# mcarrickscott/modarith

Measured on AMD Instinct MI355X. Metric: 256-bit modmul/s (2^255-19), higher is better.
Workload: dtype u64; 1 GPU; batched modmul 2^255-19, 5x51-bit limbs, 2^24 elements per GPU, limb-interleaved SoA, tiles of 4096 elements [n/4096][5][4096]; elements_per_gpu=16777216, placement_policy=single placement, no probe

## Files before the change

### include/modarith_amd.h

```cpp
#ifndef MODARITH_AMD_H
#define MODARITH_AMD_H

#include <stddef.h>
#include <stdint.h>

#ifdef __cplusplus
extern "C" {
#endif

typedef uint64_t ma_spint;

int modarith_amd_abi_version(void);
const char *modarith_amd_last_error(void);
int modarith_amd_status(void);
void modarith_amd_clear_status(void);
int modarith_amd_thread_status(void);
void modarith_amd_clear_thread_status(void);
int modarith_amd_device_count(void);
int modarith_amd_set_device(int dev);
int modarith_amd_malloc(void **dptr, size_t bytes);
int modarith_amd_free(void *dptr);
int modarith_amd_memcpy_h2d(void *dst, const void *src, size_t bytes, void *stream);
int modarith_amd_memcpy_d2h(void *dst, const void *src, size_t bytes, void *stream);
int modarith_amd_sync(void *stream);
int modarith_amd_stream_create(void **stream);
int modarith_amd_stream_destroy(void *stream);
int modarith_amd_stream_wait(void *stream, void *other);
int modarith_amd_host_alloc(void **hptr, size_t bytes);
int modarith_amd_host_free(void *hptr);
int modarith_amd_aos_to_soa(const ma_spint *aos, ma_spint *soa, size_t n, int nlimbs, size_t ld, void *stream);
int modarith_amd_soa_to_aos(const ma_spint *soa, ma_spint *aos, size_t n, int nlimbs, size_t ld, void *stream);
size_t modarith_amd_recommended_ld(size_t n);
size_t modarith_amd_recommended_ld_for(size_t n, int nlimbs);
size_t modarith_amd_batch_words(size_t n, int nlimbs, size_t ld);
int modarith_amd_scratch_trim(size_t keep_bytes);
int modarith_amd_sclk_probe(uint64_t *out, unsigned delay_us, unsigned window_us, void *stream);
int modarith_amd_wall_clock_khz(void);
const char *modarith_amd_last_launch(void);
int modarith_amd_field_info(const char *prime, int *nlimbs, int *radix, int *nbits, int *nbytes, int *montgomery);

#define MODARITH_AMD_ABI 2

#define MODARITH_AMD_DECLARE(P)                                                                                         \
                                \
    ma_spint prop_##P##_ct(ma_spint *n);            \
    ma_spint flatten_##P##_ct(ma_spint *n);                                                                             \
    ma_spint modfsb_##P##_ct(ma_spint *n);                                                                              \
    void modadd_##P##_ct(const ma_spint *a, const ma_spint *b, ma_spint *n);                                            \
    void modsub_##P##_ct(const ma_spint *a, const ma_spint *b, ma_spint *n);                                            \
    void modneg_##P##_ct(const ma_spint *b, ma_spint *n);                                                               \
    void modmli_##P##_ct(const ma_spint *a, int b, ma_spint *c);                                                        \
    void modmul_##P##_ct(const ma_spint *a, const ma_spint *b, ma_spint *c);                                            \
    void modsqr_##P##_ct(const ma_spint *a, ma_spint *c);                                                               \
    void modcpy_##P##_ct(const ma_spint *a, ma_spint *c);                                                               \
    void modnsqr_##P##_ct(ma_spint *a, int n);                                                                          \
    void modpro_##P##_ct(const ma_spint *w, ma_spint *z);                                                               \
    void modinv_##P##_ct(const ma_spint *x, const ma_spint *h, ma_spint *z);                         \
    int modqr_##P##_ct(const ma_spint *h, const ma_spint *x);                                        \
// ... 230 lines not shown
```

### modarith_amd/_lib.py

```python
from __future__ import annotations

import ctypes
import os
from ctypes import c_char_p, c_int, c_size_t, c_uint, c_void_p

HERE = os.path.dirname(os.path.abspath(__file__))
LIB_PATH = os.environ.get("MA_LIB", os.path.join(HERE, "libmodarith_amd.so"))
PRIMES = ("X25519", "NIST256", "X448",
          "NIST521", "PM266", "PM383", "NUMS256W", "NIST384", "NIST224", "SECP256K1M", "NIST256Q", "ED25519Q", "ED448Q",
          "C2065", "PM336", "PM512", "GM270", "GM240", "GM360", "GM480", "GM384", "GM512", "TWEEDLE", "SIDH434", "SIDH503",
          "SECP256K1", "C41417", "ED248", "ED376", "ED500",
          "SIDH610", "SIDH751", "MFP4", "MFP7", "MFP1973", "CSIDH512", "GM378",
          "PM383M", "PM266M", "PM336M", "C41417M", "PM512M", "M607")
LADDERS = ("X25519", "X448")
CURVES = {"ed25519": (5, 32), "ed448": (8, 56), "nist256": (5, 32), "nist384": (7, 48), "nist521": (9, 66), "secp256k1": (5, 32), "nums256w": (5, 32), "nums256e": (5, 32), "ed248": (5, 32), "ed376": (7, 48), "ed500": (9, 64)}
ED_BATCH_FUNCS = ("mul", "mul2", "mul2_exact", "ran", "add", "sub", "cpy", "dbl", "neg", "inf", "gen", "cof", "affine", "cmp", "isinf", "set", "get")
FUSED_CURVES = ("ed25519", "ed448", "nist256", "secp256k1")
FUSED2_CURVES = ("ed25519", "ed448", "nist256", "secp256k1")
FUSEDG_CURVES = ("nist256", "secp256k1", "ed25519", "ed448")
FUSEDG2_CURVES = ("nist256", "secp256k1", "ed25519", "ed448")
FUSED_FUNCS = (("rfc7748_X25519_base_batch", "rfc7748_X448_base_batch") + tuple("ecn_%s_mulgen_get_batch" % c for c in FUSEDG_CURVES)
               + tuple("ecn_%s_mulgen2_get_%s" % (c, f) for c in FUSEDG2_CURVES for f in ("batch", "workspace_bytes")) + tuple("ecn_%s_mul_get_%s" % (c, f) for c in FUSED_CURVES for f in ("batch", "workspace_bytes"))
               + tuple("ecn_%s_mul2_get_%s" % (c, f) for c in FUSED2_CURVES for f in ("batch", "workspace_bytes")))
ED_SCALAR_FUNCS = ("mul2", "ran", "get", "set", "inf", "isinf", "neg", "add", "sub", "dbl", "gen", "mul", "cmp", "affine", "cpy", "cof",
# ... 32 lines not shown
    "modsign": [_P, _P, c_size_t, c_size_t, _P],
    "modlimbs": [_P, _P, c_size_t, c_size_t, _P],
    "modcmp": [_P, _P, _P, c_size_t, c_size_t, _P],
    "modzer": [_P, c_size_t, c_size_t, _P],
    "modone": [_P, c_size_t, c_size_t, _P],
    "modint": [c_int, _P, c_size_t, c_size_t, _P],
    "mod2r": [c_uint, _P, c_size_t, c_size_t, _P],
    "modcmv": [_P, _P, _P, c_size_t, c_size_t, _P],
    "modcsw": [_P, _P, _P, c_size_t, c_size_t, _P],
    "modimp": [_P, _P, _P, c_size_t, c_size_t, _P],
    "modexp": [_P, _P, c_size_t, c_size_t, _P],
    "time_protocol": [c_int, _P, _P, _P, ctypes.c_long, c_size_t, c_size_t, _P],
    "moduniform": [ctypes.c_ulonglong, ctypes.c_ulonglong, c_size_t, c_int, _P, c_size_t, c_size_t, _P],
}
BATCH_FUNCS = tuple(_SIG)
SCALAR_FUNCS = ("prop", "flatten", "modfsb", "modadd", "modsub", "modneg", "modmli", "modmul", "modsqr", "modcpy", "modnsqr",
                "modpro", "modinv", "modqr", "modsqrt", "nres", "redc", "modis1", "modis0", "modzer", "modone", "modint", "modcmv",
                "modcsw", "modshl", "modshr", "modhaf", "mod2r", "modexp", "modimp", "modsign", "modcmp")
UTIL_FUNCS = ("modarith_amd_abi_version", "modarith_amd_last_error", "modarith_amd_device_count",
              "modarith_amd_set_device", "modarith_amd_malloc", "modarith_amd_free", "modarith_amd_memcpy_h2d",
              "modarith_amd_memcpy_d2h", "modarith_amd_sync", "modarith_amd_aos_to_soa", "modarith_amd_soa_to_aos",
              "modarith_amd_stream_create", "modarith_amd_stream_destroy", "modarith_amd_stream_wait", "modarith_amd_host_alloc", "modarith_amd_host_free",
              "modarith_amd_field_info", "modarith_amd_recommended_ld", "modarith_amd_recommended_ld_for", "modarith_amd_batch_words", "modarith_amd_scratch_trim",
              "modarith_amd_last_launch", "modarith_amd_status", "modarith_amd_clear_status", "modarith_amd_thread_status", "modarith_amd_clear_thread_status", "modarith_amd_sclk_probe", "modarith_amd_wall_clock_khz")

W32_PRIMES = ("X25519", "NIST256", "X448")
W32_ABSENT = ("modmuls", "modadd_lazy", "modsub_lazy", "modneg_lazy", "time_protocol")
_SIG_W32 = {fn: args for fn, args in _SIG.items() if fn not in W32_ABSENT}
W32_BATCH_FUNCS = tuple(_SIG_W32)
W32_SCALAR_FUNCS = SCALAR_FUNCS
W32_UTIL_FUNCS = ("modarith_amd_w32_field_info", "modarith_amd_w32_aos_to_soa", "modarith_amd_w32_soa_to_aos", "modarith_amd_w32_batch_words")
W32_CURVES = {"ed25519": (9, 32), "nist256": (9, 32), "ed448": (16, 56)}
W32_ED_BATCH_FUNCS = tuple(f for f in ED_BATCH_FUNCS if f != "mul2_exact")
W32_ED_SCALAR_FUNCS = ED_SCALAR_FUNCS


def _declare_curve(lib, C: str, funcs=ED_BATCH_FUNCS) -> None:
    g = lambda f: getattr(lib, "ecn_%s_%s" % (C, f))
    g("mul_workspace_bytes").argtypes = [c_size_t]
    g("mul_workspace_bytes").restype = c_size_t
    g("mul_batch").argtypes = [_P, _P, c_size_t, c_size_t, _P, c_size_t, _P]
    g("mul2_batch").argtypes = [_P, _P, _P, _P, _P, c_size_t, c_size_t, _P, c_size_t, _P]
    if "mul2_exact" in funcs:
        g("mul2_exact_batch").argtypes = [_P, _P, _P, _P, _P, c_size_t, c_size_t, _P, c_size_t, _P]
    g("ran_batch").argtypes = [c_int, _P, c_size_t, c_size_t, _P]
    for f in ("add", "sub", "cpy"):
        g(f + "_batch").argtypes = [_P, _P, c_size_t, c_size_t, _P]
# ... 91 lines not shown
    lib.modarith_amd_free.argtypes = [_P]
    lib.modarith_amd_memcpy_h2d.argtypes = [_P, _P, c_size_t, _P]
    lib.modarith_amd_memcpy_d2h.argtypes = [_P, _P, c_size_t, _P]
    lib.modarith_amd_sync.argtypes = [_P]
    lib.modarith_amd_stream_create.argtypes = [ctypes.POINTER(c_void_p)]
    lib.modarith_amd_stream_destroy.argtypes = [_P]
    lib.modarith_amd_stream_wait.argtypes = [_P, _P]
    lib.modarith_amd_host_alloc.argtypes = [ctypes.POINTER(c_void_p), c_size_t]
    lib.modarith_amd_host_free.argtypes = [_P]
    lib.modarith_amd_recommended_ld.argtypes = [c_size_t]
    lib.modarith_amd_recommended_ld.restype = c_size_t
    lib.modarith_amd_recommended_ld_for.argtypes = [c_size_t, c_int]
    lib.modarith_amd_recommended_ld_for.restype = c_size_t
    lib.modarith_amd_batch_words.argtypes = [c_size_t, c_int, c_size_t]
    lib.modarith_amd_batch_words.restype = c_size_t
    lib.modarith_amd_scratch_trim.argtypes = [c_size_t]
    lib.modarith_amd_scratch_trim.restype = c_int
    lib.modarith_amd_last_launch.restype = c_char_p
    lib.modarith_amd_status.restype = c_int
    lib.modarith_amd_clear_status.restype = None
    lib.modarith_amd_sclk_probe.argtypes = [_P, ctypes.c_uint, ctypes.c_uint, _P]
    lib.modarith_amd_sclk_probe.restype = c_int
    lib.modarith_amd_wall_clock_khz.restype = c_int
    _lib = lib
    return lib


_plugins = {}


def load_plugin(tag: str, path: str = None, wl: int = 64) -> ctypes.CDLL:
    if (tag, wl) in _plugins:
        return _plugins[tag, wl]
    if wl not in (64, 32):
        raise ValueError("word length must be 64 or 32")
    load()
    if path is None:
        from .generate import plugin_path
        path = plugin_path(tag, wl=wl)
    if not os.path.exists(path):
        raise RuntimeError("modarith_amd: no plug-in for %r (%s) -- generate it with `python -m modarith_amd.generate %s <prime>`. "
                           "There is no CPU fallback." % (tag, path, "64" if wl == 64 else "w32"))
    lib = ctypes.CDLL(path)
    for fn, args in (_SIG if wl == 64 else _SIG_W32).items():
        f = getattr(lib, "%s_%s%s_batch" % (fn, tag, "" if wl == 64 else "_w32"))
        f.argtypes = args
# ... 46 lines not shown
```

### modarith_amd/csrc/capi_common.h

```cpp
#pragma once
#include <hip/hip_runtime.h>
#include <mutex>
#include <stddef.h>
#include <stdint.h>
#include <stdio.h>
#include <stdlib.h>
#include <string>

namespace ma {

void set_error(const std::string& msg);
int check_launch(const char* what);
int max_blocks();
int max_blocks_tiled();
int ladder_block();
bool force_fast();
bool force_exact();
bool inv_simul();
bool ladder_split();
int scratch_trim(size_t keep_bytes);
bool ladder_use_field();

inline unsigned grid_for(size_t nthreads, int block = 256, bool tiled = false) {
    size_t b = (nthreads + (size_t)block - 1) / (size_t)block;
    size_t cap = (size_t)(tiled ? max_blocks_tiled() : max_blocks());
    if (b > cap) b = cap;
    if (b < 1) b = 1;
    return (unsigned)b;
}

inline bool aligned16(const void* p) { return (reinterpret_cast<uintptr_t>(p) & 15u) == 0; }

void fail(const char* what, hipError_t e);
int sticky_status();
void clear_sticky_status();
int thread_status();
void clear_thread_status();

struct Staging {
    static constexpr int MAX_DEVICES = 64;
    std::mutex mu[MAX_DEVICES];
    unsigned char* dev[MAX_DEVICES] = {};
    static constexpr size_t BYTES = 512 * 1024;
    unsigned char* get(int d);
};
Staging& staging();
struct StageBase {
    std::unique_lock<std::mutex> lock;
    unsigned char* base = nullptr;
    size_t used = 0;
    bool bad = false;
    struct Src { const unsigned char* p; size_t b; } src[8];
// ... 30 lines not shown
```

### modarith_amd/csrc/capi_common.hip

```cpp
#include "../../include/modarith_amd.h"
#include "capi_common.h"
#include "kernels.h"
#include <atomic>
#include <string.h>

namespace ma {

static thread_local std::string g_err;
static thread_local const char* g_last_launch = "";

void set_error(const std::string& msg) { g_err = msg; }

int check_launch(const char* what) {
    g_last_launch = what;
    hipError_t e = hipGetLastError();
    if (e != hipSuccess) {
        set_error(std::string(what) + ": " + hipGetErrorString(e));
        return (int)e;
    }
    return 0;
}

static int env_int(const char* name, int dflt, int lo, int hi) {
    const char* s = getenv(name);
// ... 16 lines not shown
    static int v = env_int("MA_LADDER_BLOCK", 64, 64, 256) / 64 * 64;
    return v;
}

bool force_fast() {
    static bool v = [] { const char* s = getenv("MA_FORCE_FAST"); return s && *s == '1'; }();
    return v;
}
bool force_exact() {
    static bool v = [] { const char* s = getenv("MA_FORCE_EXACT"); return s && *s == '1'; }();
    return v;
}
bool inv_simul() {
    static bool v = [] { const char* s = getenv("MA_INV_SIMUL"); return !(s && *s == '0'); }();
    return v;
}
bool ladder_split() {
    static bool v = [] { const char* s = getenv("MA_LADDER_SPLIT"); return !(s && *s == '0'); }();
    return v;
}
bool ladder_use_field() {
    static bool v = [] { const char* s = getenv("MA_LADDER_IMPL"); return s && strcmp(s, "field") == 0; }();
    return v;
}

static std::atomic<int> g_sticky{0};
static thread_local int t_sticky = 0;
int thread_status() { return t_sticky; }
void clear_thread_status() { t_sticky = 0; }
void fail(const char* what, hipError_t e) {
    set_error(std::string(what) + " failed: " + hipGetErrorString(e));
    int zero = 0;
    const int code = e == hipSuccess ? (int)hipErrorUnknown : (int)e;
    g_sticky.compare_exchange_strong(zero, code);
    if (t_sticky == 0) t_sticky = code;
    (void)hipGetLastError();
}
int sticky_status() { return g_sticky.load(); }
void clear_sticky_status() { g_sticky.store(0); }

unsigned char* Staging::get(int d) {
    if (!dev[d]) {
        static const bool test_fail = [] { const char* s = getenv("MA_TEST_STAGING_FAIL"); return s && *s == '1'; }();
        hipError_t e = test_fail ? hipErrorOutOfMemory : hipMalloc((void**)&dev[d], BYTES);
        if (e != hipSuccess) {
            dev[d] = nullptr;
// ... 218 lines not shown
}

extern "C" {

int modarith_amd_abi_version(void) { return MODARITH_AMD_ABI; }
const char* modarith_amd_last_error(void) { return g_err.c_str(); }
const char* modarith_amd_last_launch(void) { return g_last_launch; }
int modarith_amd_status(void) { return sticky_status(); }
void modarith_amd_clear_status(void) { clear_sticky_status(); }
int modarith_amd_thread_status(void) { return thread_status(); }
void modarith_amd_clear_thread_status(void) { clear_thread_status(); }
int modarith_amd_wall_clock_khz(void) {
    int d = 0, khz = 0;
    if (hipGetDevice(&d) != hipSuccess || hipDeviceGetAttribute(&khz, hipDeviceAttributeWallClockRate, d) != hipSuccess) { (void)hipGetLastError(); return 0; }
    return khz;
}
int modarith_amd_sclk_probe(uint64_t* out, unsigned delay_us, unsigned window_us, void* st) {
    const int khz = modarith_amd_wall_clock_khz();
    if (khz <= 0) { set_error("sclk_probe: no wall-clock rate for this device"); return (int)hipErrorNotSupported; }
    k_sclk_probe<<<1, 64, 0, (hipStream_t)st>>>(out, (uint64_t)delay_us * (uint64_t)khz / 1000, (uint64_t)window_us * (uint64_t)khz / 1000);
    return check_launch("sclk_probe");
}
int modarith_amd_scratch_trim(size_t keep_bytes) { return scratch_trim(keep_bytes); }
size_t modarith_amd_recommended_ld(size_t n) { return n >= 2 * (size_t)4096 ? (size_t)4096 : n; }
size_t modarith_amd_recommended_ld_for(size_t n, int nlimbs) {
    const size_t t = nlimbs >= 8 ? (size_t)8192 : (size_t)4096;
    return n >= 2 * t ? t : modarith_amd_recommended_ld(n);
}
size_t modarith_amd_batch_words(size_t n, int nlimbs, size_t ld) {
    if (nlimbs < 1 || ld == 0) return 0;
    if (ld >= n) return (size_t)nlimbs * ld;
    return (n + ld - 1) / ld * ld * (size_t)nlimbs;
}
int modarith_amd_device_count(void) {
    int n = 0;
    if (hipGetDeviceCount(&n) != hipSuccess) return 0;
    return n;
}
int modarith_amd_set_device(int dev) { return wrap(hipSetDevice(dev), "hipSetDevice"); }
int modarith_amd_malloc(void** dptr, size_t bytes) { return wrap(hipMalloc(dptr, bytes), "hipMalloc"); }
int modarith_amd_free(void* dptr) { return wrap(hipFree(dptr), "hipFree"); }
int modarith_amd_memcpy_h2d(void* dst, const void* src, size_t bytes, void* stream) {
    return wrap(hipMemcpyAsync(dst, src, bytes, hipMemcpyHostToDevice, (hipStream_t)stream), "hipMemcpyAsync(h2d)");
}
int modarith_amd_memcpy_d2h(void* dst, const void* src, size_t bytes, void* stream) {
    return wrap(hipMemcpyAsync(dst, src, bytes, hipMemcpyDeviceToHost, (hipStream_t)stream), "hipMemcpyAsync(d2h)");
// ... 62 lines not shown
```

### modarith_amd/csrc/capi_field.inc

```

namespace {
bool make_ld(size_t n, size_t ld, Ld* L, const char* what) {
    if (ld >= n) { *L = Ld(ld); return true; }
    if (ld < 128 || (ld & (ld - 1)) != 0) {
        set_error(std::string(what) + ": a limb stride below n selects the tiled layout and must be a power of two >= 128");
        return false;
    }
    *L = Ld(ld, (unsigned)__builtin_ctzll((unsigned long long)ld));
    return true;
}
#define GRID(x) grid_for((x), BLOCK, L.s != 63)
#define MA_LD(what)                                                  \
    Ld L;                                                            \
    if (!make_ld(n, ld, &L, what)) return (int)hipErrorInvalidValue;

uintptr_t U(const void* p) { return reinterpret_cast<uintptr_t>(p); }
int pick_ept(size_t n, size_t ld, uintptr_t addr) {
    for (int e = ept_cap(); e > 1; e >>= 1)
        if (n >= (size_t)e && ld % e == 0 && (addr & (e * sizeof(spint) - 1)) == 0) return e;
    return 1;
}
template <int E> using Width = std::integral_constant<int, E>;
#ifdef MA_W32_EPT_MAX
constexpr int EPT_COMPILED = MA_W32_EPT_MAX;
#else
constexpr int EPT_COMPILED = 4;
#endif
template <class Go>
int launch_stream(size_t n, size_t ld, uintptr_t addr, const char* what, Go go) {
    if (n == 0) return 0;
    MA_LD(what)
    const int ept = pick_ept(n, ld, addr), sb = std::min(stream_block(), stream_block_max(ept));
    const size_t nt = n / ept, done = nt * ept;
    const unsigned grid = grid_for(nt, sb, L.s != 63);
    if (ept == 4) { if constexpr (MA_WL == 32 && EPT_COMPILED >= 4) go(Width<4>{}, grid, sb, 0, nt, L); }
    else if (ept == 2) { if constexpr (EPT_COMPILED >= 2) go(Width<2>{}, grid, sb, 0, nt, L); }
    else go(Width<1>{}, grid, sb, 0, nt, L);
    if (done < n) go(Width<1>{}, 1u, BLOCK, L.off<NL>(done), n - done, Ld(L.ld));
    return check_launch(what);
}
template <class Op, int E> using OpAt = typename std::conditional<E == 1, typename ScalarOp<Op>::type, Op>::type;
template <class Op>
int launch_binary(const spint* a, const spint* b, spint* c, size_t n, size_t ld, void* stream, const char* what) {
    return launch_stream(n, ld, U(a) | U(b) | U(c), what, [=](auto W, unsigned grid, int block, size_t o, size_t cnt, Ld l) {
        constexpr int E = decltype(W)::value;
        k_binary<P, OpAt<Op, E>, E><<<grid, block, 0, (hipStream_t)stream>>>(a + o, b + o, c + o, cnt, l, l, l);
    });
}
template <class Op>
int launch_unary(const spint* a, spint* c, size_t n, size_t ld, void* stream, const char* what) {
    return launch_stream(n, ld, U(a) | U(c), what, [=](auto W, unsigned grid, int block, size_t o, size_t cnt, Ld l) {
        constexpr int E = decltype(W)::value;
        k_unary<P, OpAt<Op, E>, E><<<grid, block, 0, (hipStream_t)stream>>>(a + o, c + o, cnt, l, l);
    });
}
template <class Op>
int launch_unary_heavy(const spint* a, spint* c, size_t n, size_t ld, void* stream, const char* what) {
    if (n == 0) return 0;
    MA_LD(what)
    k_unary_heavy<P, Op><<<GRID(n), BLOCK, 0, (hipStream_t)stream>>>(a, c, n, L, L);
    return check_launch(what);
}
int modinv_each(const spint* x, spint* z, size_t n, size_t ld, void* st);
bool inv_may_share();

struct Stage : StageBase {
    template <class T>
    T* put(const T* host, size_t count) {
        T* d = reinterpret_cast<T*>(take(count * sizeof(T)));
        if (host) h2d(d, host, count * sizeof(T));
        return d;
    }
    template <class T>
    void get(T* host, const T* dev, size_t count) { d2h(host, dev, count * sizeof(T)); }
};
}

extern "C" {

int BATCH(modadd)(const spint* a, const spint* b, spint* c, size_t n, size_t ld, void* st) { return launch_binary<OpAdd<P>>(a, b, c, n, ld, st, MA_WHAT("modadd")); }
int BATCH(modsub)(const spint* a, const spint* b, spint* c, size_t n, size_t ld, void* st) { return launch_binary<OpSub<P>>(a, b, c, n, ld, st, MA_WHAT("modsub")); }
int BATCH(modneg)(const spint* b, spint* c, size_t n, size_t ld, void* st) { return launch_unary<OpNeg<P>>(b, c, n, ld, st, MA_WHAT("modneg")); }
int BATCH(modcpy)(const spint* a, spint* c, size_t n, size_t ld, void* st) { return launch_unary<OpCpy<P>>(a, c, n, ld, st, MA_WHAT("modcpy")); }
int BATCH(modmli)(const spint* a, int b, spint* c, size_t n, size_t ld, void* st) {
    return launch_stream(n, ld, U(a) | U(c), MA_WHAT("modmli"), [=](auto W, unsigned grid, int block, size_t o, size_t cnt, Ld l) {
        k_mli<P, decltype(W)::value><<<grid, block, 0, (hipStream_t)st>>>(a + o, b, c + o, cnt, l, l);
    });
}

constexpr size_t INV_SIMUL_LANES = 16384;
constexpr size_t INV_SIMUL_MIN = 32768;
int BATCH(modinv)(const spint* x, const spint* h, spint* z, size_t n, size_t ld, void* st) {
    if (n == 0) return 0;
    MA_LD(MA_WHAT("modinv"))
    if constexpr (INV_SIMUL)
    if (h == nullptr && n >= INV_SIMUL_MIN && inv_simul() && inv_may_share()) {
        hipStream_t s = (hipStream_t)st;
        size_t rounds = (n + INV_SIMUL_LANES - 1) / INV_SIMUL_LANES;
        if (rounds > 64) rounds = 64;
        const size_t lanes = (n + rounds - 1) / rounds;
        const unsigned grid = (unsigned)((lanes + BLOCK - 1) / BLOCK);
        if (x != z) {
            k_inv_simul<P><<<grid, BLOCK, 0, s>>>(x, z, z, n, lanes, (int)rounds, L, L, L);
            return check_launch(MA_WHAT2("modinv", "simultaneous"));
        }
        hipStreamCaptureStatus cs = hipStreamCaptureStatusNone;
        if (s == nullptr || (hipStreamIsCapturing(s, &cs) == hipSuccess && cs == hipStreamCaptureStatusNone)) {
            if (spint* ws = static_cast<spint*>(scratch_alloc(n * NL * sizeof(spint), s))) {
                k_inv_simul<P><<<grid, BLOCK, 0, s>>>(x, z, ws, n, lanes, (int)rounds, L, L, Ld(n));
// ... 296 lines not shown
```

### modarith_amd/csrc/capi_prime.inc

```
#include "../../include/modarith_amd.h"
#include "capi_common.h"
#include "kernels.h"
#include "ladder.h"
#ifdef MA_LADDER_FE26
#include "fe26.h"
#endif
#ifdef MA_LADDER_FE28
#include "fe28.h"
#endif
#include <string.h>
#include <algorithm>

#define MA_CAT3_(a, b, c) a##_##b##_##c
#define MA_CAT3(a, b, c) MA_CAT3_(a, b, c)
#define BATCH(fn) MA_CAT3(fn, MA_NAME, batch)
#define SCALAR(fn) MA_CAT3(fn, MA_NAME, ct)

namespace {
using namespace ma;
using P = MA_P;
constexpr int NL = P::N;
constexpr int NB = P::NBYTES;
#define MA_WHAT(fn) fn
#define MA_WHAT2(fn, how) fn "(" how ")"
int ept_cap() { return 2; }
int stream_block() { return BLOCK; }
constexpr bool INV_SIMUL = NL <= 9 && P::RADIX <= 60;
}
#include "capi_field.inc"

namespace {
int modinv_each(const spint* x, spint* z, size_t n, size_t ld, void* st) {
    if (force_fast() && P::SPLIT > 0) return launch_unary_heavy<OpInv<P, true>>(x, z, n, ld, st, "modinv(fast)");
    if (force_exact() || P::SPLIT == 0) return launch_unary_heavy<OpInv<P>>(x, z, n, ld, st, "modinv(exact)");
    return launch_unary_heavy<OpAutoUnary<P, OpInv>>(x, z, n, ld, st, "modinv");
}
bool inv_may_share() { return !force_exact(); }
template <int EPT, bool AUTO>
void launch_shared(const spint* a, const Elem<P>& b0, spint* c, size_t nt, Ld L, unsigned grid, hipStream_t s) {
    k_mul_shared<P, EPT, AUTO><<<grid, BLOCK, 0, s>>>(a, b0, c, nt, L, L);
}
}

extern "C" {

int BATCH(modadd_lazy)(const ma_spint* a, const ma_spint* b, ma_spint* c, size_t n, size_t ld, void* st) { return launch_binary<OpAddLazy<P>>(a, b, c, n, ld, st, "modadd_lazy"); }
int BATCH(modsub_lazy)(const ma_spint* a, const ma_spint* b, ma_spint* c, size_t n, size_t ld, void* st) { return launch_binary<OpSubLazy<P>>(a, b, c, n, ld, st, "modsub_lazy"); }
int BATCH(modneg_lazy)(const ma_spint* b, ma_spint* c, size_t n, size_t ld, void* st) { return launch_unary<OpNegLazy<P>>(b, c, n, ld, st, "modneg_lazy"); }
int BATCH(modmul)(const ma_spint* a, const ma_spint* b, ma_spint* c, size_t n, size_t ld, void* st) {
    if (force_fast() && P::SPLIT > 0) return launch_binary<OpMul<P, true>>(a, b, c, n, ld, st, "modmul(fast)");
    if (force_exact() || P::SPLIT == 0) return launch_binary<OpMul<P>>(a, b, c, n, ld, st, "modmul(exact)");
    return launch_binary<OpMulAuto<P>>(a, b, c, n, ld, st, "modmul");
}
int BATCH(modsqr)(const ma_spint* a, ma_spint* c, size_t n, size_t ld, void* st) {
    if (force_fast() && P::SPLIT > 0) return launch_unary<OpSqr<P, true>>(a, c, n, ld, st, "modsqr(fast)");
    if (force_exact() || P::SPLIT == 0) return launch_unary<OpSqr<P>>(a, c, n, ld, st, "modsqr(exact)");
    return launch_unary<OpSqrAuto<P>>(a, c, n, ld, st, "modsqr");
}
int BATCH(nres)(const ma_spint* a, ma_spint* c, size_t n, size_t ld, void* st) {
    if (force_fast() && P::SPLIT > 0) return launch_unary<OpNres<P, true>>(a, c, n, ld, st, "nres(fast)");
    if (force_exact() || P::SPLIT == 0 || !P::MONTGOMERY) return launch_unary<OpNres<P>>(a, c, n, ld, st, "nres(exact)");
    return launch_unary<OpNresAuto<P>>(a, c, n, ld, st, "nres");
}
// ... 15 lines not shown
        return launch_unary_heavy<OpAutoUnary<P, OpSqrt>>(x, r, n, ld, st, "modsqrt");
    }
    k_sqrt_h<P, false><<<GRID(n), BLOCK, 0, (hipStream_t)st>>>(x, h, r, nullptr, n, L);
    return check_launch("modsqrt(h)");
}
int BATCH(modqr)(const ma_spint* h, const ma_spint* x, int* out, size_t n, size_t ld, void* st) {
    if (n == 0) return 0;
    MA_LD("modqr")
    if (h == nullptr) k_inplace<P, K_MODQR><<<GRID(n), BLOCK, 0, (hipStream_t)st>>>(const_cast<ma_spint*>(x), out, n, L);
    else k_sqrt_h<P, true><<<GRID(n), BLOCK, 0, (hipStream_t)st>>>(x, h, nullptr, out, n, L);
    return check_launch("modqr");
}

int BATCH(modmuls)(const ma_spint* a, const ma_spint* b0_host, ma_spint* c, size_t n, size_t ld, void* st) {
    if (n == 0) return 0;
    Elem<P> b0;
    bool b_ok = P::SPLIT > 0 && !force_exact();
    for (int i = 0; i < NL; i++) {
        b0.l[i] = b0_host[i];
        if (P::RADIX + 2 < 64 && (b0_host[i] >> ((P::RADIX + 2) & 63)) != 0) b_ok = false;
    }
    MA_LD("modmuls")
    hipStream_t s = (hipStream_t)st;
    if (n >= 2 && ld % 2 == 0 && aligned16(a) && aligned16(c)) {
        size_t nt = n / 2;
        if (b_ok) launch_shared<2, true>(a, b0, c, nt, L, GRID(nt), s);
        else launch_shared<2, false>(a, b0, c, nt, L, GRID(nt), s);
        const size_t o = L.off<NL>(n - 1);
        if (n & 1) launch_shared<1, false>(a + o, b0, c + o, 1, Ld(L.ld), 1, s);
    } else {
        launch_shared<1, false>(a, b0, c, n, L, GRID(n), s);
    }
    return check_launch("modmuls");
}

int BATCH(time_protocol)(int kind, const ma_spint* x, const ma_spint* y, ma_spint* z, long outer, size_t n, size_t ld, void* st) {
    if (n == 0) return 0;
    MA_LD("time_protocol")
    hipStream_t s = (hipStream_t)st;
    if (kind < 0 || kind > 2) { set_error("time_protocol: kind must be 0, 1 or 2"); return (int)hipErrorInvalidValue; }
    const int policy = (P::SPLIT == 0 || force_exact()) ? 0 : (force_fast() ? 1 : 2);
#define MA_TIME_LAUNCH(KIND, POL) k_time<P, KIND, POL><<<GRID(n), BLOCK, 0, s>>>(x, y, z, outer, n, L)
    if (policy == 0) { if (kind == 0) MA_TIME_LAUNCH(0, 0); else if (kind == 1) MA_TIME_LAUNCH(1, 0); else MA_TIME_LAUNCH(2, 0); }
    else if (policy == 1) { if (kind == 0) MA_TIME_LAUNCH(0, 1); else if (kind == 1) MA_TIME_LAUNCH(1, 1); else MA_TIME_LAUNCH(2, 1); }
    else { if (kind == 0) MA_TIME_LAUNCH(0, 2); else if (kind == 1) MA_TIME_LAUNCH(1, 2); else MA_TIME_LAUNCH(2, 2); }
#undef MA_TIME_LAUNCH
    return check_launch("time_protocol");
}

#ifdef MA_LADDER_A24
#define LADDER_BATCH_(name) rfc7748_##name##_batch
#define LADDER_BATCH(name) LADDER_BATCH_(name)
#define LADDER_SCALAR_(name) rfc7748_##name
#define LADDER_SCALAR(name) LADDER_SCALAR_(name)
// ... 93 lines not shown
```

### modarith_amd/csrc/kernels.h

```cpp
#pragma once
#include "field.h"

namespace MA_NS {

constexpr int BLOCK = 256;
constexpr int stream_block_max(int ept) { return MA_WL == 32 && ept == 1 ? 512 : BLOCK; }
__device__ __forceinline__ size_t stream_threads() { if constexpr (MA_WL == 32) return blockDim.x; else return BLOCK; }

template <int EPT> struct VecOf { typedef spint type __attribute__((ext_vector_type(EPT))); };
template <> struct VecOf<1> { typedef spint type; };
typedef VecOf<2>::type spint2;
#ifndef MA_NONTEMPORAL
#define MA_NONTEMPORAL 1
#endif
template <class T> __device__ __forceinline__ T ld_stream(const T* p) {
#if MA_NONTEMPORAL
    return __builtin_nontemporal_load(p);
#else
    return *p;
#endif
}
template <class T> __device__ __forceinline__ void st_stream(T* p, T v) {
#if MA_NONTEMPORAL
    __builtin_nontemporal_store(v, p);
#else
    *p = v;
#endif
}

struct Ld {
    size_t ld;
    unsigned s;
    __host__ __device__ Ld(size_t ld_ = 0) : ld(ld_), s(63) {}
    __host__ __device__ Ld(size_t ld_, unsigned s_) : ld(ld_), s(s_) {}
    template <int N>
    __host__ __device__ __forceinline__ size_t off(size_t j) const { return (((j >> s) * (size_t)N) << s) + (j & ((((size_t)1) << s) - 1)); }
};

template <class P, int EPT>
__device__ __forceinline__ void load_soa(const spint* base, Ld L, size_t t, spint (*x)[P::N]) {
    static_assert(EPT == 1 || EPT == 2 || (EPT == 4 && MA_WL == 32), "one or two elements per lane, four of 32-bit limbs");
    const spint* p = base + L.template off<P::N>((size_t)EPT * t);
    if constexpr (EPT == 1) {
        static_for<0, P::N>([&](auto I) { x[0][I] = ld_stream(p + (size_t)I * L.ld); });
    } else {
        using V = typename VecOf<EPT>::type;
        static_for<0, P::N>([&](auto I) {
            V v = ld_stream(reinterpret_cast<const V*>(p + (size_t)I * L.ld));
            static_for<0, EPT>([&](auto E) { constexpr int e = E; x[e][I] = v[e]; });
        });
    }
}
template <class P, int EPT>
__device__ __forceinline__ void store_soa(spint* base, Ld L, size_t t, spint (*x)[P::N]) {
    spint* p = base + L.template off<P::N>((size_t)EPT * t);
    if constexpr (EPT == 1) {
        static_for<0, P::N>([&](auto I) { st_stream(p + (size_t)I * L.ld, x[0][I]); });
    } else {
        using V = typename VecOf<EPT>::type;
        static_for<0, P::N>([&](auto I) {
            V v;
            static_for<0, EPT>([&](auto E) { constexpr int e = E; v[e] = x[e][I]; });
            st_stream(reinterpret_cast<V*>(p + (size_t)I * L.ld), v);
        });
    }
}

#if MA_WL == 64
#define MA_POLICY_OP template <class P, bool FAST = false>
#define MA_POLICY_FIELD Field<P, FAST>
#else
#define MA_POLICY_OP template <class P>
#define MA_POLICY_FIELD Field<P>
#endif
template <class P> using FieldVoted = Field<P, (P::SPLIT > 0)>;
MA_POLICY_OP struct OpMul { static MA_DEV void apply(const spint* a, const spint* b, spint* c) { MA_POLICY_FIELD::modmul(a, b, c); } };
template <class P> struct OpAdd { static MA_DEV void apply(const spint* a, const spint* b, spint* c) { Field<P>::modadd(a, b, c); } };
template <class P> struct OpSub { static MA_DEV void apply(const spint* a, const spint* b, spint* c) { Field<P>::modsub(a, b, c); } };
template <class P> struct OpAddLazy { static MA_DEV void apply(const spint* a, const spint* b, spint* c) { Field<P>::modadd_lazy(a, b, c); } };
template <class P> struct OpSubLazy { static MA_DEV void apply(const spint* a, const spint* b, spint* c) { Field<P>::modsub_lazy(a, b, c); } };
template <class P> MA_DEV bool in_split_contract(const spint* a) {
    if constexpr (P::RADIX + 2 >= 64) {
        return true;
    } else {
        spint m = 0;
        static_for<0, P::N>([&](auto I) { m |= a[I]; });
        return (m >> (P::RADIX + 2)) == 0;
    }
// ... 55 lines not shown
    spint t[F::N];
    F::redc(z, t);
    F::nres(t, z);
}
MA_POLICY_OP struct OpInv {
    static MA_DEV void apply(const spint* a, spint* c) {
        MA_POLICY_FIELD::modinv(a, nullptr, c);
        inv_normalise<MA_POLICY_FIELD>(c);
    }
};
MA_POLICY_OP struct OpSqrt { static MA_DEV void apply(const spint* a, spint* c) { MA_POLICY_FIELD::modsqrt(a, nullptr, c); } };
MA_POLICY_OP struct OpPro { static MA_DEV void apply(const spint* a, spint* c) { MA_POLICY_FIELD::modpro(a, c); } };
template <class P, template <class, bool> class Op> struct OpAutoUnary {
    static MA_DEV void apply(const spint* a, spint* c) {
        if constexpr (P::SPLIT > 0) {
            if (__all(in_split_contract<P>(a))) { Op<P, true>::apply(a, c); return; }
        }
        Op<P, false>::apply(a, c);
    }
};

template <class P, class Op, int EPT>
__global__ __launch_bounds__(stream_block_max(EPT)) void k_binary(const spint* a, const spint* b,
                                                                  spint* c, size_t nthreads, Ld lda, Ld ldb, Ld ldc) {
    for (size_t t = (size_t)blockIdx.x * stream_threads() + threadIdx.x; t < nthreads; t += (size_t)gridDim.x * stream_threads()) {
        spint x[EPT][P::N], y[EPT][P::N], z[EPT][P::N];
        load_soa<P, EPT>(a, lda, t, x);
        load_soa<P, EPT>(b, ldb, t, y);
        Op::apply(x[0], y[0], z[0]);
        if constexpr (EPT >= 2) Op::apply(x[1], y[1], z[1]);
        if constexpr (EPT == 4) { Op::apply(x[2], y[2], z[2]); Op::apply(x[3], y[3], z[3]); }
        store_soa<P, EPT>(c, ldc, t, z);
    }
}

template <class P> constexpr int heavy_waves() { return (MA_WL == 32 || P::N <= 5) ? 3 : 1; }
template <class P, class Op>
__global__ __launch_bounds__(BLOCK) __attribute__((amdgpu_waves_per_eu(heavy_waves<P>())))
void k_unary_heavy(const spint* a, spint* c, size_t nthreads, Ld lda, Ld ldc) {
    for (size_t t = (size_t)blockIdx.x * BLOCK + threadIdx.x; t < nthreads; t += (size_t)gridDim.x * BLOCK) {
        spint x[1][P::N], z[1][P::N];
        load_soa<P, 1>(a, lda, t, x);
        Op::apply(x[0], z[0]);
        store_soa<P, 1>(c, ldc, t, z);
    }
}

template <class P, class Op, int EPT>
__global__ __launch_bounds__(stream_block_max(EPT)) void k_unary(const spint* a, spint* c, size_t nthreads,
                                                                 Ld lda, Ld ldc) {
    for (size_t t = (size_t)blockIdx.x * stream_threads() + threadIdx.x; t < nthreads; t += (size_t)gridDim.x * stream_threads()) {
        spint x[EPT][P::N], z[EPT][P::N];
        load_soa<P, EPT>(a, lda, t, x);
        Op::apply(x[0], z[0]);
        if constexpr (EPT >= 2) Op::apply(x[1], z[1]);
        if constexpr (EPT == 4) { Op::apply(x[2], z[2]); Op::apply(x[3], z[3]); }
        store_soa<P, EPT>(c, ldc, t, z);
    }
}

template <class P> struct Elem { spint l[P::N]; };
template <class P, bool AUTO>
MA_DEV void mul_shared_one(const spint* x, const spint* b, spint* z) {
    if constexpr (AUTO && P::SPLIT > 0) {
        if (__all(in_split_contract<P>(x))) { Field<P, true>::modmul(x, b, z); return; }
    }
    Field<P, false>::modmul(x, b, z);
}
template <class P, int EPT, bool AUTO>
__global__ __launch_bounds__(BLOCK) void k_mul_shared(const spint* a, Elem<P> b0, spint* c,
                                                      size_t nthreads, Ld lda, Ld ldc) {
    for (size_t t = (size_t)blockIdx.x * BLOCK + threadIdx.x; t < nthreads; t += (size_t)gridDim.x * BLOCK) {
        spint x[EPT][P::N], z[EPT][P::N];
        load_soa<P, EPT>(a, lda, t, x);
        static_assert(EPT == 1 || EPT == 2, "one or two elements per lane");
        mul_shared_one<P, AUTO>(x[0], b0.l, z[0]);
        if constexpr (EPT == 2) mul_shared_one<P, AUTO>(x[1], b0.l, z[1]);
        store_soa<P, EPT>(c, ldc, t, z);
    }
}

template <class P, int EPT>
__global__ __launch_bounds__(stream_block_max(EPT)) void k_mli(const spint* a, int b, spint* c, size_t nthreads,
                                                               Ld lda, Ld ldc) {
    for (size_t t = (size_t)blockIdx.x * stream_threads() + threadIdx.x; t < nthreads; t += (size_t)gridDim.x * stream_threads()) {
        spint x[EPT][P::N], z[EPT][P::N];
        load_soa<P, EPT>(a, lda, t, x);
        Field<P>::modmli(x[0], b, z[0]);
        if constexpr (EPT >= 2) Field<P>::modmli(x[1], b, z[1]);
        if constexpr (EPT == 4) { Field<P>::modmli(x[2], b, z[2]); Field<P>::modmli(x[3], b, z[3]); }
        store_soa<P, EPT>(c, ldc, t, z);
    }
}

template <class P>
__global__ __launch_bounds__(BLOCK) void k_nsqr(spint* a, int k, size_t n, Ld ld) {
    for (size_t t = (size_t)blockIdx.x * BLOCK + threadIdx.x; t < n; t += (size_t)gridDim.x * BLOCK) {
        spint x[1][P::N];
        load_soa<P, 1>(a, ld, t, x);
        if constexpr (MA_WL == 32) {
            Field<P>::modnsqr(x[0], k);
        } else {
#pragma unroll 1
            for (int i = 0; i < k; i++) {
                bool fast = false;
                if constexpr (P::SPLIT > 0) fast = __all(in_split_contract<P>(x[0]));
                if (fast) Field<P, true>::modsqr(x[0], x[0]); else Field<P, false>::modsqr(x[0], x[0]);
            }
        }
        store_soa<P, 1>(a, ld, t, x);
    }
}

template <class P>
__global__ __launch_bounds__(BLOCK) void k_inv_h(const spint* xs, const spint* hs,
// ... 347 lines not shown
```

Baseline: 54.94 billion modmul/s.

## Alternate sweep direction per call and keep the tail chunks cache-resident

Streaming kernels (binary, unary, mli, shared-multiply) now walk block-sized chunks in a direction that flips on every call, per device. By default the last ~192 MiB of chunks use ordinary temporal loads and stores instead of nontemporal ones. The intent is that the data touched last stays in the last-level cache, so the next reversed call starts on cached data and cuts DRAM traffic for memory-bound batched modmul. The benefit depends on back-to-back calls over the same buffers. The default budget is tied to a guess about cache capacity. Per-thread control flow gets slightly more complex.

```diff
diff --git a/include/modarith_amd.h b/include/modarith_amd.h
--- a/include/modarith_amd.h
+++ b/include/modarith_amd.h
@@ -34,6 +34,12 @@
 size_t modarith_amd_recommended_ld_for(size_t n, int nlimbs);
 size_t modarith_amd_batch_words(size_t n, int nlimbs, size_t ld);
 int modarith_amd_scratch_trim(size_t keep_bytes);
+int modarith_amd_set_sweep(int mode);
+int modarith_amd_get_sweep(void);
+int modarith_amd_set_sweep_policy(int policy);
+int modarith_amd_get_sweep_policy(void);
+int modarith_amd_set_sweep_keep_mib(int mib);
+int modarith_amd_get_sweep_keep_mib(void);
 int modarith_amd_sclk_probe(uint64_t *out, unsigned delay_us, unsigned window_us, void *stream);
 int modarith_amd_wall_clock_khz(void);
 const char *modarith_amd_last_launch(void);
diff --git a/modarith_amd/_lib.py b/modarith_amd/_lib.py
--- a/modarith_amd/_lib.py
+++ b/modarith_amd/_lib.py
@@ -78,7 +78,9 @@
               "modarith_amd_memcpy_d2h", "modarith_amd_sync", "modarith_amd_aos_to_soa", "modarith_amd_soa_to_aos",
               "modarith_amd_stream_create", "modarith_amd_stream_destroy", "modarith_amd_stream_wait", "modarith_amd_host_alloc", "modarith_amd_host_free",
               "modarith_amd_field_info", "modarith_amd_recommended_ld", "modarith_amd_recommended_ld_for", "modarith_amd_batch_words", "modarith_amd_scratch_trim",
-              "modarith_amd_last_launch", "modarith_amd_status", "modarith_amd_clear_status", "modarith_amd_thread_status", "modarith_amd_clear_thread_status", "modarith_amd_sclk_probe", "modarith_amd_wall_clock_khz")
+              "modarith_amd_last_launch", "modarith_amd_status", "modarith_amd_clear_status", "modarith_amd_thread_status", "modarith_amd_clear_thread_status", "modarith_amd_sclk_probe", "modarith_amd_wall_clock_khz",
+              "modarith_amd_set_sweep", "modarith_amd_get_sweep", "modarith_amd_set_sweep_policy", "modarith_amd_get_sweep_policy",
+              "modarith_amd_set_sweep_keep_mib", "modarith_amd_get_sweep_keep_mib")
 
 W32_PRIMES = ("X25519", "NIST256", "X448")
 W32_ABSENT = ("modmuls", "modadd_lazy", "modsub_lazy", "modneg_lazy", "time_protocol")
@@ -216,6 +218,11 @@
     lib.modarith_amd_sclk_probe.argtypes = [_P, ctypes.c_uint, ctypes.c_uint, _P]
     lib.modarith_amd_sclk_probe.restype = c_int
     lib.modarith_amd_wall_clock_khz.restype = c_int
+    for fn in ("set_sweep", "set_sweep_policy", "set_sweep_keep_mib"):
+        getattr(lib, "modarith_amd_" + fn).argtypes = [c_int]
+        getattr(lib, "modarith_amd_" + fn).restype = c_int
+        getattr(lib, "modarith_amd_get" + fn[3:]).argtypes = []
+        getattr(lib, "modarith_amd_get" + fn[3:]).restype = c_int
     _lib = lib
     return lib
 
diff --git a/modarith_amd/csrc/capi_common.h b/modarith_amd/csrc/capi_common.h
--- a/modarith_amd/csrc/capi_common.h
+++ b/modarith_amd/csrc/capi_common.h
@@ -28,6 +28,17 @@
     if (b < 1) b = 1;
     return (unsigned)b;
 }
+
+struct SweepChoice { size_t nchunks; size_t keep_from; unsigned reverse; };
+SweepChoice sweep_next(size_t nchunks, size_t chunk_bytes);
+int sweep_mode();
+int sweep_policy();
+int sweep_keep_mib();
+int set_sweep_mode(int mode);
+int set_sweep_policy(int policy);
+int set_sweep_keep_mib(int mib);
+template <class S> S sweep_of(const SweepChoice& c) { S s; s.nchunks = c.nchunks; s.keep_from = c.keep_from; s.reverse = c.reverse; return s; }
+template <class S> S sweep_plain(size_t nthreads, int block) { S s; s.nchunks = (nthreads + (size_t)block - 1) / (size_t)block; return s; }
 
 inline bool aligned16(const void* p) { return (reinterpret_cast<uintptr_t>(p) & 15u) == 0; }
 
diff --git a/modarith_amd/csrc/capi_common.hip b/modarith_amd/csrc/capi_common.hip
--- a/modarith_amd/csrc/capi_common.hip
+++ b/modarith_amd/csrc/capi_common.hip
@@ -62,6 +62,50 @@
 bool ladder_use_field() {
     static bool v = [] { const char* s = getenv("MA_LADDER_IMPL"); return s && strcmp(s, "field") == 0; }();
     return v;
+}
+
+static constexpr int SWEEP_MODE_DEFAULT = 1, SWEEP_POLICY_DEFAULT = 2, SWEEP_KEEP_MIB_DEFAULT = 192, SWEEP_KEEP_MIB_MAX = 1 << 20;
+static std::atomic<int>& sweep_mode_var() { static std::atomic<int> v{env_int("MA_SWEEP", SWEEP_MODE_DEFAULT, 0, 2)}; return v; }
+static std::atomic<int>& sweep_policy_var() { static std::atomic<int> v{env_int("MA_SWEEP_POLICY", SWEEP_POLICY_DEFAULT, 0, 2)}; return v; }
+static std::atomic<int>& sweep_keep_var() { static std::atomic<int> v{env_int("MA_SWEEP_KEEP_MIB", SWEEP_KEEP_MIB_DEFAULT, 0, SWEEP_KEEP_MIB_MAX)}; return v; }
+static std::atomic<unsigned> g_sweep_parity[Staging::MAX_DEVICES];
+int sweep_mode() { return sweep_mode_var().load(std::memory_order_relaxed); }
+int sweep_policy() { return sweep_policy_var().load(std::memory_order_relaxed); }
+int sweep_keep_mib() { return sweep_keep_var().load(std::memory_order_relaxed); }
+int set_sweep_mode(int mode) {
+    if (mode < 0 || mode > 2) { set_error("set_sweep: mode must be 0 (upwards), 1 (alternate) or 2 (downwards)"); return (int)hipErrorInvalidValue; }
+    sweep_mode_var().store(mode, std::memory_order_relaxed);
+    return 0;
+}
+int set_sweep_policy(int policy) {
+    if (policy < 0 || policy > 2) { set_error("set_sweep_policy: policy must be 0 (hinted), 1 (plain) or 2 (hybrid)"); return (int)hipErrorInvalidValue; }
+    sweep_policy_var().store(policy, std::memory_order_relaxed);
+    return 0;
+}
+int set_sweep_keep_mib(int mib) {
+    if (mib < 0 || mib > SWEEP_KEEP_MIB_MAX) { set_error("set_sweep_keep_mib: the budget is 0 .. 2^20 MiB"); return (int)hipErrorInvalidValue; }
+    sweep_keep_var().store(mib, std::memory_order_relaxed);
+    return 0;
+}
+SweepChoice sweep_next(size_t nchunks, size_t chunk_bytes) {
+    SweepChoice c{nchunks, ~(size_t)0, 0u};
+    const int mode = sweep_mode();
+    if (mode == 0) return c;
+    if (mode == 2) {
+        c.reverse = 1;
+    } else {
+        int d = 0;
+        if (hipGetDevice(&d) != hipSuccess || d < 0 || d >= Staging::MAX_DEVICES) { (void)hipGetLastError(); d = 0; }
+        c.reverse = g_sweep_parity[d].fetch_add(1u, std::memory_order_relaxed) & 1u;
+    }
+    const int policy = sweep_policy();
+    if (policy == 1) {
+        c.keep_from = 0;
+    } else if (policy == 2) {
+        const size_t region = chunk_bytes ? ((size_t)sweep_keep_mib() << 20) / chunk_bytes : 0;
+        c.keep_from = region >= nchunks ? 0 : nchunks - region;
+    }
+    return c;
 }
 
 static std::atomic<int> g_sticky{0};
@@ -326,6 +370,12 @@
     return check_launch("sclk_probe");
 }
 int modarith_amd_scratch_trim(size_t keep_bytes) { return scratch_trim(keep_bytes); }
+int modarith_amd_set_sweep(int mode) { return set_sweep_mode(mode); }
+int modarith_amd_get_sweep(void) { return sweep_mode(); }
+int modarith_amd_set_sweep_policy(int policy) { return set_sweep_policy(policy); }
+int modarith_amd_get_sweep_policy(void) { return sweep_policy(); }
+int modarith_amd_set_sweep_keep_mib(int mib) { return set_sweep_keep_mib(mib); }
+int modarith_amd_get_sweep_keep_mib(void) { return sweep_keep_mib(); }
 size_t modarith_amd_recommended_ld(size_t n) { return n >= 2 * (size_t)4096 ? (size_t)4096 : n; }
 size_t modarith_amd_recommended_ld_for(size_t n, int nlimbs) {
     const size_t t = nlimbs >= 8 ? (size_t)8192 : (size_t)4096;
diff --git a/modarith_amd/csrc/capi_field.inc b/modarith_amd/csrc/capi_field.inc
--- a/modarith_amd/csrc/capi_field.inc
+++ b/modarith_amd/csrc/capi_field.inc
@@ -27,31 +27,32 @@
 constexpr int EPT_COMPILED = 4;
 #endif
 template <class Go>
-int launch_stream(size_t n, size_t ld, uintptr_t addr, const char* what, Go go) {
+int launch_stream(size_t n, size_t ld, uintptr_t addr, int streams, const char* what, Go go) {
     if (n == 0) return 0;
     MA_LD(what)
     const int ept = pick_ept(n, ld, addr), sb = std::min(stream_block(), stream_block_max(ept));
     const size_t nt = n / ept, done = nt * ept;
     const unsigned grid = grid_for(nt, sb, L.s != 63);
-    if (ept == 4) { if constexpr (MA_WL == 32 && EPT_COMPILED >= 4) go(Width<4>{}, grid, sb, 0, nt, L); }
-    else if (ept == 2) { if constexpr (EPT_COMPILED >= 2) go(Width<2>{}, grid, sb, 0, nt, L); }
-    else go(Width<1>{}, grid, sb, 0, nt, L);
-    if (done < n) go(Width<1>{}, 1u, BLOCK, L.off<NL>(done), n - done, Ld(L.ld));
+    const Sweep sw = sweep_of<Sweep>(sweep_next((nt + (size_t)sb - 1) / (size_t)sb, (size_t)streams * NL * sizeof(spint) * (size_t)ept * (size_t)sb));
+    if (ept == 4) { if constexpr (MA_WL == 32 && EPT_COMPILED >= 4) go(Width<4>{}, grid, sb, 0, nt, L, sw); }
+    else if (ept == 2) { if constexpr (EPT_COMPILED >= 2) go(Width<2>{}, grid, sb, 0, nt, L, sw); }
+    else go(Width<1>{}, grid, sb, 0, nt, L, sw);
+    if (done < n) go(Width<1>{}, 1u, BLOCK, L.off<NL>(done), n - done, Ld(L.ld), sweep_plain<Sweep>(n - done, BLOCK));
     return check_launch(what);
 }
 template <class Op, int E> using OpAt = typename std::conditional<E == 1, typename ScalarOp<Op>::type, Op>::type;
 template <class Op>
 int launch_binary(const spint* a, const spint* b, spint* c, size_t n, size_t ld, void* stream, const char* what) {
-    return launch_stream(n, ld, U(a) | U(b) | U(c), what, [=](auto W, unsigned grid, int block, size_t o, size_t cnt, Ld l) {
+    return launch_stream(n, ld, U(a) | U(b) | U(c), 3, what, [=](auto W, unsigned grid, int block, size_t o, size_t cnt, Ld l, Sweep sw) {
         constexpr int E = decltype(W)::value;
-        k_binary<P, OpAt<Op, E>, E><<<grid, block, 0, (hipStream_t)stream>>>(a + o, b + o, c + o, cnt, l, l, l);
+        k_binary<P, OpAt<Op, E>, E><<<grid, block, 0, (hipStream_t)stream>>>(a + o, b + o, c + o, cnt, l, l, l, sw);
     });
 }
 template <class Op>
 int launch_unary(const spint* a, spint* c, size_t n, size_t ld, void* stream, const char* what) {
-    return launch_stream(n, ld, U(a) | U(c), what, [=](auto W, unsigned grid, int block, size_t o, size_t cnt, Ld l) {
+    return launch_stream(n, ld, U(a) | U(c), 2, what, [=](auto W, unsigned grid, int block, size_t o, size_t cnt, Ld l, Sweep sw) {
         constexpr int E = decltype(W)::value;
-        k_unary<P, OpAt<Op, E>, E><<<grid, block, 0, (hipStream_t)stream>>>(a + o, c + o, cnt, l, l);
+        k_unary<P, OpAt<Op, E>, E><<<grid, block, 0, (hipStream_t)stream>>>(a + o, c + o, cnt, l, l, sw);
     });
 }
 template <class Op>
@@ -83,8 +84,8 @@
 int BATCH(modneg)(const spint* b, spint* c, size_t n, size_t ld, void* st) { return launch_unary<OpNeg<P>>(b, c, n, ld, st, MA_WHAT("modneg")); }
 int BATCH(modcpy)(const spint* a, spint* c, size_t n, size_t ld, void* st) { return launch_unary<OpCpy<P>>(a, c, n, ld, st, MA_WHAT("modcpy")); }
 int BATCH(modmli)(const spint* a, int b, spint* c, size_t n, size_t ld, void* st) {
-    return launch_stream(n, ld, U(a) | U(c), MA_WHAT("modmli"), [=](auto W, unsigned grid, int block, size_t o, size_t cnt, Ld l) {
-        k_mli<P, decltype(W)::value><<<grid, block, 0, (hipStream_t)st>>>(a + o, b, c + o, cnt, l, l);
+    return launch_stream(n, ld, U(a) | U(c), 2, MA_WHAT("modmli"), [=](auto W, unsigned grid, int block, size_t o, size_t cnt, Ld l, Sweep sw) {
+        k_mli<P, decltype(W)::value><<<grid, block, 0, (hipStream_t)st>>>(a + o, b, c + o, cnt, l, l, sw);
     });
 }
 
diff --git a/modarith_amd/csrc/capi_prime.inc b/modarith_amd/csrc/capi_prime.inc
--- a/modarith_amd/csrc/capi_prime.inc
+++ b/modarith_amd/csrc/capi_prime.inc
@@ -37,8 +37,8 @@
 }
 bool inv_may_share() { return !force_exact(); }
 template <int EPT, bool AUTO>
-void launch_shared(const spint* a, const Elem<P>& b0, spint* c, size_t nt, Ld L, unsigned grid, hipStream_t s) {
-    k_mul_shared<P, EPT, AUTO><<<grid, BLOCK, 0, s>>>(a, b0, c, nt, L, L);
+void launch_shared(const spint* a, const Elem<P>& b0, spint* c, size_t nt, Ld L, unsigned grid, hipStream_t s, Sweep sw) {
+    k_mul_shared<P, EPT, AUTO><<<grid, BLOCK, 0, s>>>(a, b0, c, nt, L, L, sw);
 }
 }
 
@@ -100,14 +100,18 @@
     }
     MA_LD("modmuls")
     hipStream_t s = (hipStream_t)st;
+    const auto sweep = [&](size_t nt, int ept) {
+        return sweep_of<Sweep>(sweep_next((nt + BLOCK - 1) / BLOCK, (size_t)2 * NL * sizeof(spint) * (size_t)ept * BLOCK));
+    };
     if (n >= 2 && ld % 2 == 0 && aligned16(a) && aligned16(c)) {
         size_t nt = n / 2;
-        if (b_ok) launch_shared<2, true>(a, b0, c, nt, L, GRID(nt), s);
-        else launch_shared<2, false>(a, b0, c, nt, L, GRID(nt), s);
+        const Sweep sw = sweep(nt, 2);
+        if (b_ok) launch_shared<2, true>(a, b0, c, nt, L, GRID(nt), s, sw);
+        else launch_shared<2, false>(a, b0, c, nt, L, GRID(nt), s, sw);
         const size_t o = L.off<NL>(n - 1);
-        if (n & 1) launch_shared<1, false>(a + o, b0, c + o, 1, Ld(L.ld), 1, s);
+        if (n & 1) launch_shared<1, false>(a + o, b0, c + o, 1, Ld(L.ld), 1, s, sweep_plain<Sweep>(1, BLOCK));
     } else {
-        launch_shared<1, false>(a, b0, c, n, L, GRID(n), s);
+        launch_shared<1, false>(a, b0, c, n, L, GRID(n), s, sweep(n, 1));
     }
     return check_launch("modmuls");
 }
diff --git a/modarith_amd/csrc/kernels.h b/modarith_amd/csrc/kernels.h
--- a/modarith_amd/csrc/kernels.h
+++ b/modarith_amd/csrc/kernels.h
@@ -13,19 +13,17 @@
 #ifndef MA_NONTEMPORAL
 #define MA_NONTEMPORAL 1
 #endif
-template <class T> __device__ __forceinline__ T ld_stream(const T* p) {
+template <bool NT = true, class T> __device__ __forceinline__ T ld_stream(const T* p) {
 #if MA_NONTEMPORAL
-    return __builtin_nontemporal_load(p);
-#else
+    if constexpr (NT) return __builtin_nontemporal_load(p);
+#endif
     return *p;
+}
+template <bool NT = true, class T> __device__ __forceinline__ void st_stream(T* p, T v) {
+#if MA_NONTEMPORAL
+    if constexpr (NT) { __builtin_nontemporal_store(v, p); return; }
 #endif
-}
-template <class T> __device__ __forceinline__ void st_stream(T* p, T v) {
-#if MA_NONTEMPORAL
-    __builtin_nontemporal_store(v, p);
-#else
     *p = v;
-#endif
 }
 
 struct Ld {
@@ -37,33 +35,56 @@
     __host__ __device__ __forceinline__ size_t off(size_t j) const { return (((j >> s) * (size_t)N) << s) + (j & ((((size_t)1) << s) - 1)); }
 };
 
-template <class P, int EPT>
+template <class P, int EPT, bool NT = true>
 __device__ __forceinline__ void load_soa(const spint* base, Ld L, size_t t, spint (*x)[P::N]) {
     static_assert(EPT == 1 || EPT == 2 || (EPT == 4 && MA_WL == 32), "one or two elements per lane, four of 32-bit limbs");
     const spint* p = base + L.template off<P::N>((size_t)EPT * t);
     if constexpr (EPT == 1) {
-        static_for<0, P::N>([&](auto I) { x[0][I] = ld_stream(p + (size_t)I * L.ld); });
+        static_for<0, P::N>([&](auto I) { x[0][I] = ld_stream<NT>(p + (size_t)I * L.ld); });
     } else {
         using V = typename VecOf<EPT>::type;
         static_for<0, P::N>([&](auto I) {
-            V v = ld_stream(reinterpret_cast<const V*>(p + (size_t)I * L.ld));
+            V v = ld_stream<NT>(reinterpret_cast<const V*>(p + (size_t)I * L.ld));
             static_for<0, EPT>([&](auto E) { constexpr int e = E; x[e][I] = v[e]; });
         });
     }
 }
-template <class P, int EPT>
+template <class P, int EPT, bool NT = true>
 __device__ __forceinline__ void store_soa(spint* base, Ld L, size_t t, spint (*x)[P::N]) {
     spint* p = base + L.template off<P::N>((size_t)EPT * t);
     if constexpr (EPT == 1) {
-        static_for<0, P::N>([&](auto I) { st_stream(p + (size_t)I * L.ld, x[0][I]); });
+        static_for<0, P::N>([&](auto I) { st_stream<NT>(p + (size_t)I * L.ld, x[0][I]); });
     } else {
         using V = typename VecOf<EPT>::type;
         static_for<0, P::N>([&](auto I) {
             V v;
             static_for<0, EPT>([&](auto E) { constexpr int e = E; v[e] = x[e][I]; });
-            st_stream(reinterpret_cast<V*>(p + (size_t)I * L.ld), v);
+            st_stream<NT>(reinterpret_cast<V*>(p + (size_t)I * L.ld), v);
         });
     }
+}
+
+struct Sweep {
+    size_t nchunks = 0;
+    size_t keep_from = ~(size_t)0;
+    unsigned reverse = 0;
+};
+template <class F>
+__device__ __forceinline__ void sweep_chunks(size_t nthreads, size_t T, const Sweep& sw, F f) {
+    for (size_t q = blockIdx.x; q < sw.nchunks; q += gridDim.x) {
+        const size_t c = sw.reverse ? sw.nchunks - 1 - q : q;
+        const size_t t = c * T + threadIdx.x;
+        if (t < nthreads) f(t, q >= sw.keep_from);
+    }
+}
+#define MA_KEEP_APART() asm volatile("" ::: "memory")
+template <class P, int EPT>
+__device__ __forceinline__ void load_soa_sw(const spint* base, Ld L, size_t t, spint (*x)[P::N], bool keep) {
+    if (keep) { MA_KEEP_APART(); load_soa<P, EPT, false>(base, L, t, x); MA_KEEP_APART(); } else load_soa<P, EPT, true>(base, L, t, x);
+}
+template <class P, int EPT>
+__device__ __forceinline__ void store_soa_sw(spint* base, Ld L, size_t t, spint (*x)[P::N], bool keep) {
+    if (keep) { MA_KEEP_APART(); store_soa<P, EPT, false>(base, L, t, x); MA_KEEP_APART(); } else store_soa<P, EPT, true>(base, L, t, x);
 }
 
 #if MA_WL == 64
@@ -165,16 +186,16 @@
 
 template <class P, class Op, int EPT>
 __global__ __launch_bounds__(stream_block_max(EPT)) void k_binary(const spint* a, const spint* b,
-                                                                  spint* c, size_t nthreads, Ld lda, Ld ldb, Ld ldc) {
-    for (size_t t = (size_t)blockIdx.x * stream_threads() + threadIdx.x; t < nthreads; t += (size_t)gridDim.x * stream_threads()) {
+                                                                  spint* c, size_t nthreads, Ld lda, Ld ldb, Ld ldc, Sweep sw) {
+    sweep_chunks(nthreads, stream_threads(), sw, [&](size_t t, bool keep) {
         spint x[EPT][P::N], y[EPT][P::N], z[EPT][P::N];
-        load_soa<P, EPT>(a, lda, t, x);
-        load_soa<P, EPT>(b, ldb, t, y);
+        if (keep) { MA_KEEP_APART(); load_soa<P, EPT, false>(a, lda, t, x); load_soa<P, EPT, false>(b, ldb, t, y); MA_KEEP_APART(); }
+        else { load_soa<P, EPT, true>(a, lda, t, x); load_soa<P, EPT, true>(b, ldb, t, y); }
         Op::apply(x[0], y[0], z[0]);
         if constexpr (EPT >= 2) Op::apply(x[1], y[1], z[1]);
         if constexpr (EPT == 4) { Op::apply(x[2], y[2], z[2]); Op::apply(x[3], y[3], z[3]); }
-        store_soa<P, EPT>(c, ldc, t, z);
-    }
+        store_soa_sw<P, EPT>(c, ldc, t, z, keep);
+    });
 }
 
 template <class P> constexpr int heavy_waves() { return (MA_WL == 32 || P::N <= 5) ? 3 : 1; }
@@ -191,15 +212,15 @@
 
 template <class P, class Op, int EPT>
 __global__ __launch_bounds__(stream_block_max(EPT)) void k_unary(const spint* a, spint* c, size_t nthreads,
-                                                                 Ld lda, Ld ldc) {
-    for (size_t t = (size_t)blockIdx.x * stream_threads() + threadIdx.x; t < nthreads; t += (size_t)gridDim.x * stream_threads()) {
+                                                                 Ld lda, Ld ldc, Sweep sw) {
+    sweep_chunks(nthreads, stream_threads(), sw, [&](size_t t, bool keep) {
         spint x[EPT][P::N], z[EPT][P::N];
-        load_soa<P, EPT>(a, lda, t, x);
+        load_soa_sw<P, EPT>(a, lda, t, x, keep);
         Op::apply(x[0], z[0]);
         if constexpr (EPT >= 2) Op::apply(x[1], z[1]);
         if constexpr (EPT == 4) { Op::apply(x[2], z[2]); Op::apply(x[3], z[3]); }
-        store_soa<P, EPT>(c, ldc, t, z);
-    }
+        store_soa_sw<P, EPT>(c, ldc, t, z, keep);
+    });
 }
 
 template <class P> struct Elem { spint l[P::N]; };
@@ -212,28 +233,28 @@
 }
 template <class P, int EPT, bool AUTO>
 __global__ __launch_bounds__(BLOCK) void k_mul_shared(const spint* a, Elem<P> b0, spint* c,
-                                                      size_t nthreads, Ld lda, Ld ldc) {
-    for (size_t t = (size_t)blockIdx.x * BLOCK + threadIdx.x; t < nthreads; t += (size_t)gridDim.x * BLOCK) {
+                                                      size_t nthreads, Ld lda, Ld ldc, Sweep sw) {
+    sweep_chunks(nthreads, BLOCK, sw, [&](size_t t, bool keep) {
         spint x[EPT][P::N], z[EPT][P::N];
-        load_soa<P, EPT>(a, lda, t, x);
+        load_soa_sw<P, EPT>(a, lda, t, x, keep);
         static_assert(EPT == 1 || EPT == 2, "one or two elements per lane");
         mul_shared_one<P, AUTO>(x[0], b0.l, z[0]);
         if constexpr (EPT == 2) mul_shared_one<P, AUTO>(x[1], b0.l, z[1]);
-        store_soa<P, EPT>(c, ldc, t, z);
-    }
+        store_soa_sw<P, EPT>(c, ldc, t, z, keep);
+    });
 }
 
 template <class P, int EPT>
 __global__ __launch_bounds__(stream_block_max(EPT)) void k_mli(const spint* a, int b, spint* c, size_t nthreads,
-                                                               Ld lda, Ld ldc) {
-    for (size_t t = (size_t)blockIdx.x * stream_threads() + threadIdx.x; t < nthreads; t += (size_t)gridDim.x * stream_threads()) {
+                                                               Ld lda, Ld ldc, Sweep sw) {
+    sweep_chunks(nthreads, stream_threads(), sw, [&](size_t t, bool keep) {
         spint x[EPT][P::N], z[EPT][P::N];
-        load_soa<P, EPT>(a, lda, t, x);
+        load_soa_sw<P, EPT>(a, lda, t, x, keep);
         Field<P>::modmli(x[0], b, z[0]);
         if constexpr (EPT >= 2) Field<P>::modmli(x[1], b, z[1]);
         if constexpr (EPT == 4) { Field<P>::modmli(x[2], b, z[2]); Field<P>::modmli(x[3], b, z[3]); }
-        store_soa<P, EPT>(c, ldc, t, z);
-    }
+        store_soa_sw<P, EPT>(c, ldc, t, z, keep);
+    });
 }
 
 template <class P>
```

Result: no change. 55.26 billion modmul/s, median of 6 (+0.6%).
